# dflaxx/3d-hashjoin

Hardware: AMD Instinct MI355X
Metric: probe tuples/s + build ms, exp1 key/FK |R|=1e7 |S|=1e8, 1/2/4/8 GPU (higher is better)
Workload: dtype u32; 1 GPU; exp1 key/FK plan Csr, |R|=10000000 |S|=100000000 per GPU, uniform FKs, b=1; config=B, plan=Csr, R_total=10000000, S_total=100000000, R_per_gpu=10000000, S_per_gpu=100000000, num_buckets=10000000, emit_pairs=True, parallelism=single GPU, rehearsal_one_gpu=False

## Files before the change

3d-hashjoin_amd/csrc/radix.hip:

```cpp
#include <cmath>

#include "radix_seg.hpp"

namespace hj3d {
namespace {

constexpr int kPBlock = 1024;
constexpr int kPRounds = 16;
constexpr int kPTile = kPBlock * kPRounds;
constexpr int kPRoundsR = 8;
constexpr int kPSeg = 16;
__device__ __forceinline__ void put(uint2* p, uint2 e) { *p = e; }
__device__ __forceinline__ void put(uint32_t* p, uint32_t v) { *p = v; }
static_assert(kPTile == 1 << 14, "k_rp_scatter packs (partition, rank) as p << 14 | rank");
constexpr uint32_t kMaxParts = 2048;
constexpr uint32_t kBuildSlice = 16384;
constexpr uint32_t kSortedMax = 32;

struct FastDiv {
  uint64_t m;
  static FastDiv make(uint32_t d) {
    FastDiv f;
    f.m = ~uint64_t(0) / d + 1;
    f.d1 = d == 1;
    return f;
  }
  __device__ __forceinline__ uint32_t div(uint32_t a) const { return d1 ? a : uint32_t(__umul64hi(m, uint64_t(a))); }
  bool d1 = false;
};

struct RelTiles {
  RelView r0, r1;
  uint32_t nt0;
  uint32_t P;
  uint32_t tsz = kPTile;
  __device__ __forceinline__ bool second(uint32_t tile) const { return tile >= nt0; }
  __device__ __forceinline__ const RelView& rel(uint32_t tile) const { return tile >= nt0 ? r1 : r0; }
  __device__ __forceinline__ uint64_t base(uint32_t tile) const {
    return uint64_t(tile >= nt0 ? tile - nt0 : tile) * tsz;
  }
  __device__ __forceinline__ uint32_t pofs(uint32_t tile) const { return tile >= nt0 ? P : 0u; }
};

template <int ROUNDS>
__global__ __launch_bounds__(kPBlock) void k_rp_hist(RelTiles rt, FastMod fm, uint32_t lo, uint32_t nbl, FastDiv fw,
                                                     uint32_t P, uint32_t ntiles, uint32_t* __restrict__ hist,
                                                     uint32_t* __restrict__ cur) {
  __shared__ uint32_t cnt[kMaxParts];
  for (uint32_t p = threadIdx.x; p < P; p += kPBlock) cnt[p] = 0;
  __syncthreads();
  uint32_t key[ROUNDS];
  auto load = [&](uint32_t tile) __attribute__((always_inline)) {
    const RelView& r = rt.rel(tile);
    const uint64_t b = rt.base(tile);
#pragma unroll
    for (int j = 0; j < ROUNDS; ++j) {
      const uint64_t i = b + uint64_t(j) * kPBlock + threadIdx.x;
      key[j] = tile < ntiles && i < r.n ? r.key(i) : 0u;
    }
  };
  load(blockIdx.x);
  for (uint32_t tile = blockIdx.x; tile < ntiles; tile += gridDim.x) {
    const RelView& r = rt.rel(tile);
    const uint64_t b = rt.base(tile);
    const uint32_t pofs = rt.pofs(tile);
    uint32_t bl[ROUNDS];
#pragma unroll
    for (int j = 0; j < ROUNDS; ++j) {
      const uint64_t i = b + uint64_t(j) * kPBlock + threadIdx.x;
      bl[j] = i < r.n ? fm.mod(murmur32(key[j])) - lo : nbl;
    }
    load(tile + gridDim.x);
#pragma unroll
    for (int j = 0; j < ROUNDS; ++j)
      if (bl[j] < nbl) atomicAdd(&cnt[pofs + fw.div(bl[j])], 1u);
  }
  __syncthreads();
  for (uint32_t p = threadIdx.x; p < P; p += kPBlock) {
    const uint32_t c = cnt[p];
    hist[uint64_t(blockIdx.x) * P + p] = c ? atomicAdd(&cur[p], c) : 0u;
  }
}

template <int BLOCK = kJBlock>
__device__ uint32_t lds_excl_scan(uint32_t* a, uint32_t n, uint32_t* wsum);

template <int ROUNDS>
__global__ __launch_bounds__(kPBlock) void k_rp_scatter(RelTiles rt, FastMod fm, uint32_t lo, uint32_t nbl, FastDiv fw,
                                                        uint32_t P, uint32_t ntiles, const uint32_t* __restrict__ offs,
                                                        const uint32_t* __restrict__ cur, uint32_t* __restrict__ cur_next,
                                                        uint32_t* __restrict__ ps, uint2* __restrict__ out) {
  constexpr int kTile = kPBlock * ROUNDS;
  __shared__ uint2 stage[kTile];
  __shared__ uint32_t loc[kMaxParts];
  __shared__ uint32_t gb[kMaxParts];
  uint32_t* wsum = reinterpret_cast<uint32_t*>(stage);
  const bool explicit_rows = rt.r0.row_off != 0xFFFFFFFFu;
  uint32_t h[ROUNDS], rw[ROUNDS];
  auto load = [&](uint32_t tile) __attribute__((always_inline)) {
    const RelView& r = rt.rel(tile);
    const uint64_t b = rt.base(tile);
#pragma unroll
    for (int j = 0; j < ROUNDS; ++j) {
      const uint64_t i = b + uint64_t(j) * kPBlock + threadIdx.x;
      const bool ok = tile < ntiles && i < r.n;
      h[j] = ok ? r.key(i) : 0u;
      rw[j] = explicit_rows && ok ? r.row(i) : 0u;
    }
  };
  load(blockIdx.x);
  for (uint32_t p = threadIdx.x; p < P; p += kPBlock) gb[p] = cur[p];
  __syncthreads();
  const uint32_t total = lds_excl_scan<kPBlock>(gb, P, wsum);
  for (uint32_t p = threadIdx.x; p < P; p += kPBlock) {
    if (blockIdx.x == 0) ps[p] = gb[p];
    gb[p] += offs[uint64_t(blockIdx.x) * P + p];
  }
  if (blockIdx.x == 0) {
    if (threadIdx.x == 0) ps[P] = total;
    for (uint32_t p = threadIdx.x; p <= kMaxParts; p += kPBlock) cur_next[p] = 0;
  }
  for (uint32_t tile = blockIdx.x; tile < ntiles; tile += gridDim.x) {
    for (uint32_t p = threadIdx.x; p < P; p += kPBlock) loc[p] = 0;
    const RelView& r = rt.rel(tile);
    const uint64_t base = rt.base(tile);
    const uint32_t pofs = rt.pofs(tile);
    uint32_t rk[ROUNDS];
    __syncthreads();
#pragma unroll
    for (int j = 0; j < ROUNDS; ++j) {
      const uint64_t i = base + uint64_t(j) * kPBlock + threadIdx.x;
      h[j] = murmur32(h[j]);
      const uint32_t bl = fm.mod(h[j]) - lo;
      if (i < r.n && bl < nbl) {
        const uint32_t part = pofs + fw.div(bl);
        rk[j] = (part << 14) | atomicAdd(&loc[part], 1u);
      } else {
        rk[j] = kInvalid;
      }
    }
    __syncthreads();
    const uint32_t m = lds_excl_scan(loc, P, wsum);
#pragma unroll
    for (int j = 0; j < ROUNDS; ++j) {
      if (rk[j] == kInvalid) continue;
      const uint64_t i = base + uint64_t(j) * kPBlock + threadIdx.x;
      stage[loc[rk[j] >> 14] + (rk[j] & (kTile - 1))] = make_uint2(h[j], explicit_rows ? rw[j] : r.row(i));
    }
    __syncthreads();
    load(tile + gridDim.x);
    for (uint32_t k = threadIdx.x; k < m; k += kPBlock) {
      const uint2 e = stage[k];
      const uint32_t p = pofs + fw.div(fm.mod(e.x) - lo);
      put(out + gb[p] + (k - loc[p]), e);
    }
    __syncthreads();
    for (uint32_t p = threadIdx.x; p < P; p += kPBlock)
      gb[p] += (p + 1 < P ? loc[p + 1] : m) - loc[p];
    __syncthreads();
  }
}

constexpr int kFzRounds = 8;
constexpr int kFzGroup = 2;
constexpr int kFzTMax = 6;
struct FzBar {
  uint64_t* bar;
  uint64_t target;
  uint64_t* tflag;
  uint64_t tag;
  uint64_t ticks;
  uint32_t skip0;
};
__device__ __forceinline__ void grid_barrier(const FzBar& b) {
  __syncthreads();
  if (threadIdx.x == 0) {
    if (!(b.skip0 && blockIdx.x == 0)) __hip_atomic_fetch_add(b.bar, 1ull, __ATOMIC_RELEASE, __HIP_MEMORY_SCOPE_AGENT);
    const uint64_t t0 = wall_clock64();
    while (__hip_atomic_load(b.bar, __ATOMIC_ACQUIRE, __HIP_MEMORY_SCOPE_AGENT) < b.target) {
      __builtin_amdgcn_s_sleep(2);
      if (wall_clock64() - t0 > b.ticks) {
        __hip_atomic_store(b.bar + 1, 1ull, __ATOMIC_RELAXED, __HIP_MEMORY_SCOPE_AGENT);
        __hip_atomic_store(b.tflag, b.tag, __ATOMIC_RELAXED, __HIP_MEMORY_SCOPE_AGENT);
        break;
      }
    }
  }
  __syncthreads();
}

struct FzGeom {
  FastDiv32 dnb, dw;
  uint32_t nb, lo, nbl, P;
  __device__ __forceinline__ uint32_t bucket(uint32_t h) const { return h - dnb.div(h) * nb - lo; }
};
template <int TMAX>
__global__ __launch_bounds__(kPBlock) void k_rp_fused(RelTiles rt, FzGeom fz, uint32_t ntiles, uint32_t* __restrict__ cur,
                                                      uint32_t* __restrict__ cur_next, uint32_t* __restrict__ ps,
                                                      uint2* __restrict__ out, FzBar fb) {
  constexpr int R = kFzRounds;
  constexpr int kTile = kPBlock * R;
  __shared__ uint2 stage[kTile * kFzGroup];
  __shared__ uint32_t loc[kMaxParts];
  __shared__ uint32_t gb[kMaxParts];
  uint32_t* wsum = reinterpret_cast<uint32_t*>(stage);
  const uint32_t G = gridDim.x, P = fz.P, me = threadIdx.x;
  uint32_t hv[TMAX][R];
  for (uint32_t p = me; p < P; p += kPBlock) loc[p] = 0;
  const auto nleft = [&](uint32_t tile) __attribute__((always_inline)) {
    const RelView& r = rt.rel(tile);
    const uint64_t b = rt.base(tile);
    return tile < ntiles && r.n > b ? uint32_t(min(r.n - b, uint64_t(kTile))) : 0u;
  };
#pragma unroll
  for (int t = 0; t < TMAX; ++t) {
    const uint32_t tile = blockIdx.x + uint32_t(t) * G;
    const RelView& r = rt.rel(tile);
    const uint32_t nl = nleft(tile);
    const char* tb = r.base + rt.base(tile) * r.stride + r.key_off;
#pragma unroll
    for (int j = 0; j < R; ++j) {
      const uint32_t li = uint32_t(j) * kPBlock + me;
      hv[t][j] = li < nl ? (*reinterpret_cast<const uint32_t*>(tb + li * r.stride))
                         : 0u;
    }
  }
  __syncthreads();
#pragma unroll
  for (int t = 0; t < TMAX; ++t) {
    const uint32_t tile = blockIdx.x + uint32_t(t) * G;
    const uint32_t nl = nleft(tile), pofs = rt.pofs(tile);
#pragma unroll
    for (int j = 0; j < R; ++j) {
      hv[t][j] = murmur32(hv[t][j]);
      const uint32_t bl = fz.bucket(hv[t][j]);
      if (uint32_t(j) * kPBlock + me < nl && bl < fz.nbl) atomicAdd(&loc[pofs + fz.dw.div(bl)], 1u);
    }
  }
  __syncthreads();
  for (uint32_t p = me; p < P; p += kPBlock) {
    const uint32_t c = loc[p];
    gb[p] = c ? atomicAdd(&cur[p], c) : 0u;
  }
  grid_barrier(fb);
  for (uint32_t p = me; p < P; p += kPBlock) loc[p] = __hip_atomic_load(cur + p, __ATOMIC_RELAXED, __HIP_MEMORY_SCOPE_AGENT);
  __syncthreads();
  const uint32_t total = lds_excl_scan<kPBlock>(loc, P, wsum);
  for (uint32_t p = me; p < P; p += kPBlock) {
    if (blockIdx.x == 0) ps[p] = loc[p];
    gb[p] += loc[p];
  }
  if (blockIdx.x == 0) {
    if (me == 0) ps[P] = total;
    for (uint32_t p = me; p <= kMaxParts; p += kPBlock) cur_next[p] = 0;
  }
#pragma unroll
  for (int t0 = 0; t0 < TMAX; t0 += kFzGroup) {
    if (blockIdx.x + uint32_t(t0) * G >= ntiles) break;
    __syncthreads();
    for (uint32_t p = me; p < P; p += kPBlock) loc[p] = 0;
    uint32_t rk[kFzGroup][R];
    __syncthreads();
#pragma unroll
    for (int u = 0; u < kFzGroup; ++u) {
      const int t = t0 + u < TMAX ? t0 + u : TMAX - 1;
      const uint32_t nl = t0 + u < TMAX ? nleft(blockIdx.x + uint32_t(t) * G) : 0u;
#pragma unroll
      for (int j = 0; j < R; ++j) {
        asm volatile("" : "+v"(hv[t][j]));
        const uint32_t bl = fz.bucket(hv[t][j]);
        rk[u][j] = kInvalid;
        if (uint32_t(j) * kPBlock + me < nl && bl < fz.nbl) {
          const uint32_t part = fz.dw.div(bl);
          rk[u][j] = (part << 15) | atomicAdd(&loc[part], 1u);
        }
      }
    }
    __syncthreads();
    const uint32_t m = lds_excl_scan<kPBlock>(loc, P, wsum);
#pragma unroll
    for (int u = 0; u < kFzGroup; ++u) {
      const int t = t0 + u < TMAX ? t0 + u : TMAX - 1;
      const uint32_t rb = uint32_t(rt.r0.row_base + rt.base(blockIdx.x + uint32_t(t) * G));
#pragma unroll
      for (int j = 0; j < R; ++j) {
        if (rk[u][j] == kInvalid) continue;
        stage[loc[rk[u][j] >> 15] + (rk[u][j] & 0x7FFFu)] = make_uint2(hv[t][j], rb + uint32_t(j) * kPBlock + me);
      }
    }
    __syncthreads();
    for (uint32_t k = me; k < m; k += kPBlock) {
      const uint2 e = stage[k];
      const uint32_t p = fz.dw.div(fz.bucket(e.x));
      put(out + gb[p] + (k - loc[p]), e);
    }
    __syncthreads();
    for (uint32_t p = me; p < P; p += kPBlock) gb[p] += (p + 1 < P ? loc[p + 1] : m) - loc[p];
  }
}

constexpr uint32_t kRpWsMin = 4;
constexpr int kRpSmallRounds = 8;
constexpr int kWsRounds = 8;
constexpr int kWsSub = kPBlock * kWsRounds;
template <int PPT>
struct WsGeom {
  static constexpr uint32_t kSeg = PPT == 1 ? 16u : 8u;
  static constexpr uint32_t kStage = PPT == 1 ? 17408u : 15360u;
};
template <int PPT, bool EXPL>
__global__ __launch_bounds__(kPBlock) void k_rp_wscatter(RelTiles rt, FastMod fm, uint32_t lo, uint32_t nbl, FastDiv fw,
                                                         uint32_t P, uint32_t ntiles, const uint32_t* __restrict__ offs,
                                                         const uint32_t* __restrict__ cur, uint32_t* __restrict__ cur_next,
                                                         uint32_t* __restrict__ ps, uint2* __restrict__ out) {
  constexpr uint32_t SEG = WsGeom<PPT>::kSeg, STAGE = WsGeom<PPT>::kStage;
  __shared__ uint2 stage[STAGE];
  __shared__ uint32_t loc[kPBlock * PPT];
  __shared__ uint32_t sbase[kPBlock * PPT];
  __shared__ uint2 seginfo[STAGE / SEG];
  __shared__ uint32_t wsum[kPBlock / kWave];
  const uint32_t me = threadIdx.x;
  const int lane = threadIdx.x & 63, wid = threadIdx.x >> 6;
  for (uint32_t p = me; p < P; p += kPBlock) loc[p] = cur[p];
  __syncthreads();
  const uint32_t total = lds_excl_scan<kPBlock>(loc, P, wsum);
  if (blockIdx.x == 0) {
    for (uint32_t p = me; p < P; p += kPBlock) ps[p] = loc[p];
    if (me == 0) ps[P] = total;
    for (uint32_t p = me; p <= kMaxParts; p += kPBlock) cur_next[p] = 0;
  }
  uint32_t my_cur[PPT], my_kc[PPT], my_skip[PPT];
  uint2 creg[PPT][SEG - 1];
#pragma unroll
  for (int k = 0; k < PPT; ++k) {
    const uint32_t p = me + k * kPBlock;
    const uint32_t st = p < P ? loc[p] + offs[uint64_t(blockIdx.x) * P + p] : 0u;
    my_skip[k] = st % SEG;
    my_cur[k] = st - my_skip[k];
    my_kc[k] = my_skip[k];
#pragma unroll
    for (int j = 0; j < int(SEG) - 1; ++j) creg[k][j] = make_uint2(0, 0);
  }
  __syncthreads();
  for (uint32_t p = me; p < kPBlock * PPT; p += kPBlock) loc[p] = 0;
  __syncthreads();
  uint32_t h[kWsRounds], rw[EXPL ? kWsRounds : 1];
  auto load = [&](uint32_t tile, uint32_t hf) __attribute__((always_inline)) {
    const RelView& r = rt.rel(tile);
    const uint64_t base = rt.base(tile) + uint64_t(hf) * kWsSub;
#pragma unroll
    for (int j = 0; j < kWsRounds; ++j) {
      const uint64_t i = base + uint64_t(j) * kPBlock + me;
      h[j] = i < r.n ? r.key(i) : 0u;
      if constexpr (EXPL) rw[j] = i < r.n ? r.row(i) : 0u;
    }
  };
  auto flush_carry = [&]() __attribute__((always_inline)) {
#pragma unroll
    for (int k = 0; k < PPT; ++k) {
#pragma unroll
      for (int j = 0; j < int(SEG) - 1; ++j)
        if (uint32_t(j) < my_kc[k] && uint32_t(j) >= my_skip[k]) out[my_cur[k] + j] = creg[k][j];
      my_cur[k] += my_kc[k];
      my_kc[k] = 0;
      my_skip[k] = 0;
    }
  };
  auto scan = [&](uint32_t v, uint32_t* tot) __attribute__((always_inline)) {
    uint32_t wt;
    const uint32_t pre = wave_excl_scan(v, &wt);
    if (lane == 0) wsum[wid] = wt;
    __syncthreads();
    uint32_t base = 0, all = 0;
#pragma unroll
    for (int w = 0; w < kPBlock / kWave; ++w) {
      const uint32_t t = wsum[w];
      base += w < wid ? t : 0u;
      all += t;
    }
    __syncthreads();
    *tot = all;
    return base + pre;
  };
  auto process = [&](uint32_t tile, uint32_t hf, uint32_t ntile, uint32_t nhf) __attribute__((always_inline)) {
    const RelView& r = rt.rel(tile);
    const uint64_t base = rt.base(tile) + uint64_t(hf) * kWsSub;
    const uint32_t pofs = rt.pofs(tile);
    uint32_t rk[kWsRounds];
#pragma unroll
    for (int j = 0; j < kWsRounds; ++j) {
      const uint64_t i = base + uint64_t(j) * kPBlock + me;
      h[j] = murmur32(h[j]);
      const uint32_t bl = fm.mod(h[j]) - lo;
      rk[j] = kInvalid;
      if (i < r.n && bl < nbl) {
        const uint32_t p = pofs + fw.div(bl);
        rk[j] = (p << 13) | atomicAdd(&loc[p], 1u);
      }
    }
    __syncthreads();
    uint32_t c[PPT], L[PPT], pack = 0;
#pragma unroll
    for (int k = 0; k < PPT; ++k) {
      const uint32_t p = me + k * kPBlock;
      c[k] = p < P ? loc[p] : 0u;
      loc[p] = 0;
      L[k] = my_kc[k] + c[k];
      pack += (L[k] << 16) | (L[k] / SEG);
    }
    uint32_t tot;
    uint32_t pre = scan(pack, &tot);
    if ((tot >> 16) > STAGE) {
      flush_carry();
      pack = 0;
#pragma unroll
      for (int k = 0; k < PPT; ++k) {
        L[k] = c[k];
        pack += (L[k] << 16) | (L[k] / SEG);
      }
      pre = scan(pack, &tot);
    }
    const uint32_t nfull = tot & 0xFFFFu;
    uint32_t at = pre >> 16, fseg = pre & 0xFFFFu;
#pragma unroll
    for (int k = 0; k < PPT; ++k) {
      const uint32_t p = me + k * kPBlock;
      if (p < P) {
        sbase[p] = at + my_kc[k];
#pragma unroll
        for (int j = 0; j < int(SEG) - 1; ++j)
          if (uint32_t(j) < my_kc[k]) stage[at + j] = creg[k][j];
        for (uint32_t sg = 0; sg < L[k] / SEG; ++sg)
          seginfo[fseg + sg] = make_uint2(my_cur[k] + sg * SEG, (at + sg * SEG) | ((sg == 0 ? my_skip[k] : 0u) << 16));
      }
      at += L[k];
      fseg += L[k] / SEG;
    }
    __syncthreads();
#pragma unroll
    for (int j = 0; j < kWsRounds; ++j) {
      if (rk[j] == kInvalid) continue;
      const uint64_t i = base + uint64_t(j) * kPBlock + me;
      uint32_t row;
      if constexpr (EXPL) row = rw[j];
      else row = uint32_t(r.row_base + i);
      stage[sbase[rk[j] >> 13] + (rk[j] & (kWsSub - 1))] = make_uint2(h[j], row);
    }
    if (ntile < ntiles) load(ntile, nhf);
    __syncthreads();
    for (uint32_t kk = me; kk < nfull * SEG; kk += kPBlock) {
      const uint2 si = seginfo[kk / SEG];
      const uint32_t j = kk % SEG;
      const uint2 e = stage[(si.y & 0xFFFFu) + j];
      if (j >= (si.y >> 16)) put(out + si.x + j, e);
    }
    at = pre >> 16;
#pragma unroll
    for (int k = 0; k < PPT; ++k) {
      const uint32_t F = L[k] - L[k] % SEG;
#pragma unroll
      for (int j = 0; j < int(SEG) - 1; ++j)
        if (uint32_t(j) < L[k] - F) creg[k][j] = stage[at + F + j];
      if (F) my_skip[k] = 0;
      my_cur[k] += F;
      my_kc[k] = L[k] - F;
      at += L[k];
    }
  };
  if (blockIdx.x < ntiles) load(blockIdx.x, 0);
  for (uint32_t tile = blockIdx.x; tile < ntiles; tile += gridDim.x) {
    process(tile, 0, tile, 1);
    process(tile, 1, tile + gridDim.x, 0);
  }
  flush_carry();
}

template <int BLOCK>
__device__ uint32_t lds_excl_scan(uint32_t* a, uint32_t n, uint32_t* wsum) {
  const uint32_t per = (n + BLOCK - 1) / BLOCK;
  const uint32_t beg = threadIdx.x * per;
  const uint32_t end = min(beg + per, n);
  uint32_t local = 0;
  for (uint32_t k = beg; k < end; ++k) local += a[k];
  const int lane = threadIdx.x & 63, wid = threadIdx.x >> 6;
  uint32_t x = local;
#pragma unroll
  for (int o = 1; o < 64; o <<= 1) {
    const uint32_t y = __shfl_up(x, o, kWave);
    if (lane >= o) x += y;
  }
  if (lane == 63) wsum[wid] = x;
  __syncthreads();
  uint32_t wpre = 0, tot = 0;
  for (int w = 0; w < BLOCK / kWave; ++w) {
    const uint32_t v = wsum[w];
    if (w < wid) wpre += v;
    tot += v;
  }
  uint32_t run = wpre + x - local;
  for (uint32_t k = beg; k < end; ++k) {
    const uint32_t v = a[k];
    a[k] = run;
    run += v;
  }
  __syncthreads();
  return tot;
}

__global__ __launch_bounds__(kJBlock) void k_rp_build(const uint2* __restrict__ pairs, const uint32_t* __restrict__ ps,
                                                      FastMod fm, uint32_t lo, uint32_t nbl, uint32_t W,
                                                      uint32_t* __restrict__ off, uint2* __restrict__ ent) {
  __shared__ uint32_t cnt[kBuildSlice];
  __shared__ uint32_t wsum[kJBlock / kWave];
  const uint32_t p = blockIdx.x;
  const uint32_t b0 = p * W;
  const uint32_t nbs = min(W, nbl - b0);
  const uint32_t s0 = ps[p], s1 = ps[p + 1];
  for (uint32_t k = threadIdx.x; k < nbs; k += kJBlock) cnt[k] = 0;
  __syncthreads();
  for (uint32_t i = s0 + threadIdx.x; i < s1; i += kJBlock) atomicAdd(&cnt[fm.mod(pairs[i].x) - lo - b0], 1u);
  __syncthreads();
  lds_excl_scan(cnt, nbs, wsum);
  for (uint32_t k = threadIdx.x; k < nbs; k += kJBlock) off[b0 + k] = s0 + cnt[k];
  if (b0 + nbs == nbl && threadIdx.x == 0) off[nbl] = s1;
  __syncthreads();
  for (uint32_t i = s0 + threadIdx.x; i < s1; i += kJBlock) {
    const uint2 e = pairs[i];
    const uint32_t pos = atomicAdd(&cnt[fm.mod(e.x) - lo - b0], 1u);
    ent[s0 + pos] = e;
  }
}

constexpr uint32_t kBuildSlice2 = 8192;
constexpr uint32_t kBuildSlice2Max = 10240;
constexpr uint32_t kBuildStage = 14400;

constexpr int kB3Per = 12;
template <int BLOCK, uint32_t WMAX, uint32_t STAGE>
__global__ __launch_bounds__(BLOCK) void k_rp_build3(const uint2* __restrict__ pairs, const uint32_t* __restrict__ ps,
                                                     FastMod fm, uint32_t lo, uint32_t nbl, uint32_t W, uint32_t P,
                                                     uint32_t* __restrict__ off, uint2* __restrict__ ent) {
  __shared__ uint32_t cnt[WMAX + 1];
  __shared__ uint2 stage[STAGE];
  __shared__ uint32_t wsum[BLOCK / kWave];
  constexpr uint32_t kCap = kB3Per * BLOCK;
  static_assert(kCap <= STAGE, "a register-held partition must fit the stage");
  uint2 ea[kB3Per], eb[kB3Per];
  auto load = [&](uint2 (&e)[kB3Per], uint32_t p) __attribute__((always_inline)) {
    if (p >= P) return;
    const uint32_t s0 = ps[p], s1 = ps[p + 1];
    if (s1 - s0 > kCap) return;
#pragma unroll
    for (int u = 0; u < kB3Per; ++u) {
      const uint32_t i = s0 + u * BLOCK + threadIdx.x;
      e[u] = i < s1 ? pairs[i] : make_uint2(0, 0);
    }
  };
  auto build = [&](uint2 (&e)[kB3Per], uint32_t p) __attribute__((always_inline)) {
    const uint32_t b0 = p * W;
    const uint32_t nbs = min(W, nbl - b0);
    const uint32_t s0 = ps[p], s1 = ps[p + 1], m = s1 - s0;
    for (uint32_t k = threadIdx.x; k < nbs; k += BLOCK) cnt[k] = 0;
    __syncthreads();
    if (m > kCap) {
      for (uint32_t i = s0 + threadIdx.x; i < s1; i += BLOCK) atomicAdd(&cnt[fm.mod(pairs[i].x) - lo - b0], 1u);
      __syncthreads();
      lds_excl_scan<BLOCK>(cnt, nbs, wsum);
      for (uint32_t k = threadIdx.x; k < nbs; k += BLOCK) off[b0 + k] = s0 + cnt[k];
      if (b0 + nbs == nbl && threadIdx.x == 0) off[nbl] = s1;
      __syncthreads();
      for (uint32_t i = s0 + threadIdx.x; i < s1; i += BLOCK) {
        const uint2 x = pairs[i];
        ent[s0 + atomicAdd(&cnt[fm.mod(x.x) - lo - b0], 1u)] = x;
      }
      __syncthreads();
      for (uint32_t k = threadIdx.x; k < nbs; k += BLOCK) {
        const uint32_t bs = k ? cnt[k - 1] : 0u, n = cnt[k] - bs;
        if (n < 2 || n > kSortedMax) continue;
        uint2* E = ent + s0 + bs;
        for (uint32_t q = 1; q < n; ++q) {
          const uint2 x = E[q];
          uint32_t j = q;
          while (j > 0 && E[j - 1].y > x.y) {
            E[j] = E[j - 1];
            --j;
          }
          E[j] = x;
        }
      }
      __syncthreads();
      return;
    }
    uint32_t rk[kB3Per];
#pragma unroll
    for (int u = 0; u < kB3Per; ++u) {
      const bool v = u * BLOCK + threadIdx.x < m;
      const uint32_t b = v ? fm.mod(e[u].x) - lo - b0 : 0u;
      rk[u] = v ? (b << 16) | atomicAdd(&cnt[b], 1u) : kInvalid;
    }
    __syncthreads();
    lds_excl_scan<BLOCK>(cnt, nbs, wsum);
    if (threadIdx.x == 0) cnt[nbs] = m;
    for (uint32_t k = threadIdx.x; k < nbs; k += BLOCK) put(off + b0 + k, s0 + cnt[k]);
    if (b0 + nbs == nbl && threadIdx.x == 0) off[nbl] = s1;
    __syncthreads();
#pragma unroll
    for (int u = 0; u < kB3Per; ++u)
      if (rk[u] != kInvalid) stage[cnt[rk[u] >> 16] + (rk[u] & 0xFFFFu)] = e[u];
    __syncthreads();
    for (uint32_t q = threadIdx.x; q < m; q += BLOCK) {
      const uint2 x = stage[q];
      const uint32_t b = fm.mod(x.x) - lo - b0;
      const uint32_t bs = cnt[b], n = cnt[b + 1] - bs;
      uint32_t pos = q;
      if (n >= 2 && n <= kSortedMax) {
        uint32_t r = 0;
        for (uint32_t k = bs; k < bs + n; ++k) r += stage[k].y < x.y;
        pos = bs + r;
      }
      put(ent + s0 + pos, x);
    }
    __syncthreads();
  };
  load(ea, blockIdx.x);
  for (uint32_t p = blockIdx.x; p < P; p += 2 * gridDim.x) {
    load(eb, p + gridDim.x);
    build(ea, p);
    if (p + gridDim.x >= P) break;
    load(ea, p + 2 * gridDim.x);
    build(eb, p + gridDim.x);
  }
}

enum Mode { kAgg = 0, kDense = 1, kCount = 2, kWrite = 3 };

template <bool UNIQUE, int MODE, bool CK, typename EntT>
__device__ __forceinline__ void probe_bucket(uint32_t h, uint32_t pr, const EntT* E, uint32_t s, uint32_t n,
                                             uint64_t (&acc)[kProbeFields], uint64_t i, uint2* __restrict__ out,
                                             uint64_t out_cap, uint64_t* __restrict__ cnt) {
  if (MODE != kWrite) acc[0] += 1;
  if (UNIQUE) {
    uint32_t match = kInvalid, cmps = 0;
    if (n <= kSortedMax) {
      cmps = n;
      for (uint32_t c = 0; c < n; ++c) {
        const uint2 e = E[s + (c == 0 ? 0u : n - c)];
        if (e.x == h) {
          cmps = c + 1;
          match = e.y;
          break;
        }
      }
    } else {
      uint32_t minrow = kInvalid, lo_m = kInvalid, hi_m = 0, nm = 0;
      for (uint32_t k = s; k < s + n; ++k) {
        const uint2 e = E[k];
        minrow = min(minrow, e.y);
        if (e.x == h) {
          ++nm;
          lo_m = min(lo_m, e.y);
          hi_m = max(hi_m, e.y);
        }
      }
      if (nm == 0) {
        cmps = n;
      } else if (lo_m == minrow) {
        cmps = 1;
        match = lo_m;
      } else {
        uint32_t gt = 0;
        for (uint32_t k = s; k < s + n; ++k) gt += E[k].y > hi_m;
        cmps = 2 + gt;
        match = hi_m;
      }
    }
    if (MODE != kWrite) acc[3] += cmps;
    if (MODE == kDense) {
      if (i < out_cap)
        __builtin_nontemporal_store((uint64_t(match) << 32) | pr, reinterpret_cast<uint64_t*>(out + i));
    }
    if (match != kInvalid) {
      if (MODE == kWrite) {
        const uint64_t o = cnt[i];
        if (o < out_cap) out[o] = make_uint2(pr, match);
      } else {
        acc[1] += 1;
        acc[2] += 1;
        if (CK) {
          acc[4] += pr;
          acc[5] += match;
          const uint64_t ph = pair_hash(pr, match);
          acc[7] += ph;
          acc[8] ^= ph;
        }
      }
    }
    if (MODE == kCount) cnt[i] = match != kInvalid;
  } else {
    if (MODE != kWrite) acc[3] += n;
    uint64_t o = (MODE == kWrite) ? cnt[i] : 0;
    uint32_t nout = 0;
    for (uint32_t k = s; k < s + n; ++k) {
      const uint2 e = E[k];
      if (e.x != h) continue;
      ++nout;
      if (MODE == kWrite) {
        if (o < out_cap) out[o] = make_uint2(pr, e.y);
        ++o;
      } else if (CK) {
        acc[4] += pr;
        acc[5] += e.y;
        const uint64_t ph = pair_hash(pr, e.y);
        acc[7] += ph;
        acc[8] ^= ph;
      }
    }
    if (MODE != kWrite) {
      acc[1] += nout != 0;
      acc[2] += nout;
    }
    if (MODE == kCount) cnt[i] = nout;
  }
}

template <int MODE, bool CK, int NG>
__device__ __forceinline__ void probe_group_unique(const uint64_t (&v)[kSegItems], const uint64_t (&slot)[kSegItems],
                                                   uint32_t valid, int g, const uint32_t* loff, const uint2* lent,
                                                   FastMod fm, uint32_t lob0, uint64_t (&acc)[kProbeFields],
                                                   uint2* __restrict__ out, uint64_t out_cap) {
  static_assert(MODE == kDense || MODE == kAgg, "unique dense / aggregate forms only");
  uint32_t d[NG], match[NG], cmps[NG];
  bool live[NG];
#pragma unroll
  for (int j = 0; j < NG; ++j) {
    const bool ok = (valid >> (g + j)) & 1u;
    const uint32_t w = loff[ok ? fm.mod(uint32_t(v[g + j])) - lob0 : 0u];
    d[j] = ok ? w : 0u;
  }
#pragma unroll
  for (int j = 0; j < NG; ++j) {
    const uint32_t n = d[j] & 0xFFFFu;
    match[j] = kInvalid;
    cmps[j] = n;
    live[j] = n != 0 && n <= kSortedMax;
  }
#pragma unroll
  for (uint32_t c = 0; c < 3; ++c) {
    uint2 e[NG];
#pragma unroll
    for (int j = 0; j < NG; ++j) {
      const uint32_t n = d[j] & 0xFFFFu;
      const bool ok = live[j] && c < n;
      e[j] = lent[ok ? (d[j] >> 16) + (c == 0 ? 0u : n - c) : 0u];
      const bool hit = ok && e[j].x == uint32_t(v[g + j]);
      match[j] = hit ? e[j].y : match[j];
      cmps[j] = hit ? c + 1 : cmps[j];
      live[j] = live[j] && !hit;
    }
  }
#pragma unroll
  for (int j = 0; j < NG; ++j) {
    const uint32_t h = uint32_t(v[g + j]), n = d[j] & 0xFFFFu, s = d[j] >> 16;
    if (live[j] && n > 3) {
      for (uint32_t c = 3; c < n; ++c) {
        const uint2 e = lent[s + n - c];
        if (e.x == h) {
          cmps[j] = c + 1;
          match[j] = e.y;
          break;
        }
      }
    } else if (n > kSortedMax) {
      uint32_t minrow = kInvalid, lo_m = kInvalid, hi_m = 0, nm = 0;
      for (uint32_t k = s; k < s + n; ++k) {
        const uint2 e = lent[k];
        minrow = min(minrow, e.y);
        if (e.x == h) {
          ++nm;
          lo_m = min(lo_m, e.y);
          hi_m = max(hi_m, e.y);
        }
      }
      if (nm != 0 && lo_m == minrow) {
        cmps[j] = 1;
        match[j] = lo_m;
      } else if (nm != 0) {
        uint32_t gt = 0;
        for (uint32_t k = s; k < s + n; ++k) gt += lent[k].y > hi_m;
        cmps[j] = 2 + gt;
        match[j] = hi_m;
      }
    }
  }
  uint32_t nv = 0, nm = 0, sc = 0;
#pragma unroll
  for (int j = 0; j < NG; ++j) {
    const bool ok = (valid >> (g + j)) & 1u;
    const uint32_t pr = uint32_t(v[g + j] >> 32);
    nv += ok;
    sc += cmps[j];
    const bool m = match[j] != kInvalid;
    nm += m;
    if (MODE == kDense && ok && slot[g + j] < out_cap)
      __builtin_nontemporal_store((uint64_t(match[j]) << 32) | pr, reinterpret_cast<uint64_t*>(out + slot[g + j]));
    if (CK && m) {
      acc[4] += pr;
      acc[5] += match[j];
      const uint64_t ph = pair_hash(pr, match[j]);
      acc[7] += ph;
      acc[8] ^= ph;
    }
  }
  acc[0] += nv;
  acc[1] += nm;
  acc[2] += nm;
  acc[3] += sc;
}

template <int MODE, bool CK, int NG = 4>
__device__ __forceinline__ void probe_chunk_unique(const uint64_t (&v)[kSegItems], const uint64_t (&slot)[kSegItems],
                                                   uint32_t valid, const uint32_t* loff, const uint2* lent,
                                                   FastMod fm, uint32_t lob0, uint64_t (&acc)[kProbeFields],
                                                   uint2* __restrict__ out, uint64_t out_cap) {
  static_assert(kSegItems % NG == 0, "groups of NG items");
#pragma unroll
  for (int g = 0; g < kSegItems; g += NG)
    probe_group_unique<MODE, CK, NG>(v, slot, valid, g, loff, lent, fm, lob0, acc, out, out_cap);
}
__device__ __forceinline__ void stage_slice(const uint32_t* __restrict__ off, const uint2* __restrict__ ent, uint32_t b0,
                                            uint32_t nbs, uint32_t e0, uint32_t ne, uint32_t* ldir, uint2* lent) {
  constexpr int kStage = 12;
  const uint64_t* src = reinterpret_cast<const uint64_t*>(ent + e0);
  uint64_t* dst = reinterpret_cast<uint64_t*>(lent);
  const uint32_t nmax = max(nbs, ne);
  for (uint32_t k0 = threadIdx.x; k0 < nmax; k0 += kJBlock * kStage) {
    uint32_t v[kStage], w[kStage];
    uint64_t x[kStage];
#pragma unroll
    for (int u = 0; u < kStage; ++u) {
      const uint32_t k = k0 + u * kJBlock;
      v[u] = k < nbs ? off[b0 + k] : 0u;
      w[u] = k < nbs ? off[b0 + k + 1] : 0u;
      x[u] = k < ne ? src[k] : 0ull;
    }
#pragma unroll
    for (int u = 0; u < kStage; ++u) {
      const uint32_t k = k0 + u * kJBlock;
      if (k < nbs) ldir[k] = ((v[u] - e0) << 16) | (w[u] - v[u]);
      if (k < ne) dst[k] = x[u];
    }
  }
}

template <int BLOCK, int ROUNDS, int MAXP, bool IMPLICIT>
__global__ __launch_bounds__(BLOCK) void k_rp_part1(RelView r, FastMod fm, uint32_t lo, uint32_t nbl, FastDiv fw,
                                                    uint32_t P, uint32_t ntiles, uint32_t cap,
                                                    uint2* __restrict__ region, uint32_t* __restrict__ counts,
                                                    uint2* __restrict__ ovf, unsigned long long* __restrict__ novf) {
  constexpr int TILE = BLOCK * ROUNDS;
  constexpr int TBITS = __builtin_ctz(TILE);
  static_assert((TILE & (TILE - 1)) == 0 && TILE <= (1 << 16), "tile must be a power of two");
  static_assert(MAXP < (1 << 16), "partition ids are packed into 16 bits");
  __shared__ uint2 stage[TILE];
  __shared__ uint32_t loc[MAXP + 1];
  __shared__ uint32_t cur[MAXP];
  __shared__ uint32_t wsum[BLOCK / kWave];
  const uint64_t gbase = uint64_t(blockIdx.x) * P;
  for (uint32_t p = threadIdx.x; p < P; p += BLOCK) cur[p] = 0;
  uint32_t h[ROUNDS];
  uint32_t rw[IMPLICIT ? 1 : ROUNDS];
#pragma unroll
  for (int j = 0; j < ROUNDS; ++j) {
    const uint64_t i = uint64_t(blockIdx.x) * TILE + uint64_t(j) * BLOCK + threadIdx.x;
    h[j] = i < r.n ? r.key(i) : 0u;
    if constexpr (!IMPLICIT) rw[j] = i < r.n ? r.row(i) : 0u;
  }
  const int lane = threadIdx.x & 63;
  const uint64_t lt = lane == 0 ? 0ull : (~0ull >> (64 - lane));
  for (uint32_t tile = blockIdx.x; tile < ntiles; tile += gridDim.x) {
    for (uint32_t p = threadIdx.x; p < P; p += BLOCK) loc[p] = 0;
    const uint64_t base = uint64_t(tile) * TILE;
    uint32_t rk[ROUNDS];
    __syncthreads();
#pragma unroll
    for (int j = 0; j < ROUNDS; ++j) {
      const uint64_t i = base + uint64_t(j) * BLOCK + threadIdx.x;
      h[j] = murmur32(h[j]);
      const uint32_t bl = fm.mod(h[j]) - lo;
      if (i < r.n && bl < nbl) {
        const uint32_t part = fw.div(bl);
        rk[j] = (part << TBITS) | atomicAdd(&loc[part], 1u);
      } else {
        rk[j] = kInvalid;
      }
    }
    __syncthreads();
    const uint32_t m = lds_excl_scan<BLOCK>(loc, P, wsum);
    if (threadIdx.x == 0) loc[P] = m;
#pragma unroll
    for (int j = 0; j < ROUNDS; ++j) {
      if (rk[j] == kInvalid) continue;
      const uint32_t li = uint32_t(j) * BLOCK + threadIdx.x;
      uint32_t y = ((rk[j] >> TBITS) << 16) | li;
      if constexpr (!IMPLICIT) y = rw[j];
      stage[loc[rk[j] >> TBITS] + (rk[j] & (TILE - 1))] = make_uint2(h[j], y);
    }
    __syncthreads();
    const uint64_t nbase = uint64_t(tile + gridDim.x) * TILE;
#pragma unroll
    for (int j = 0; j < ROUNDS; ++j) {
      const uint64_t i = nbase + uint64_t(j) * BLOCK + threadIdx.x;
      h[j] = i < r.n ? r.key(i) : 0u;
      if constexpr (!IMPLICIT) rw[j] = i < r.n ? r.row(i) : 0u;
    }
    constexpr int kOutU = 4;
    for (uint32_t k0 = 0; k0 < m; k0 += kOutU * BLOCK) {
      uint2 e[kOutU];
      uint32_t o[kOutU], p[kOutU];
#pragma unroll
      for (int u = 0; u < kOutU; ++u) {
        const uint32_t k = k0 + u * BLOCK + threadIdx.x;
        e[u] = k < m ? stage[k] : make_uint2(0, 0);
      }
#pragma unroll
      for (int u = 0; u < kOutU; ++u) {
        const uint32_t k = k0 + u * BLOCK + threadIdx.x;
        if (IMPLICIT) {
          p[u] = e[u].y >> 16;
          e[u].y = uint32_t(r.row_base + base) + (e[u].y & 0xFFFFu);
        } else {
          p[u] = fw.div(fm.mod(e[u].x) - lo);
        }
        o[u] = k < m ? cur[p[u]] + (k - loc[p[u]]) : 0u;
      }
// ... 670 lines not shown
```

Baseline: 121.2 billion probe tuples/s.

## Rank all tiles once in fused partition kernel and overlap local scan with grid barrier

The fused radix-partition kernel now records each element's block-local rank during the first counting pass, packed as 16-bit slots in registers. It splits the grid barrier into arrive and wait so the local exclusive scan and slot finalisation run while other workgroups arrive. The old per-group recount and rescan is replaced by scattering into the shared stage through fixed-size windows. It also adds compile-time-disabled wall-clock instrumentation in the fused and build kernels. The cost is more register pressure from the packed slot arrays and an extra LDS array for global starts.

```diff
diff --git a/3d-hashjoin_amd/csrc/radix.hip b/3d-hashjoin_amd/csrc/radix.hip
--- a/3d-hashjoin_amd/csrc/radix.hip
+++ b/3d-hashjoin_amd/csrc/radix.hip
@@ -16,6 +16,35 @@
 constexpr uint32_t kMaxParts = 2048;
 constexpr uint32_t kBuildSlice = 16384;
 constexpr uint32_t kSortedMax = 32;
+
+#ifndef HJ3D_RP_CLK
+#define HJ3D_RP_CLK 0
+#endif
+constexpr int kRpClkPts = 32;
+#if HJ3D_RP_CLK
+#define RP_CLK_DECL __shared__ uint64_t rp_clk[kRpClkPts]
+#define RP_CLK(i)                                   \
+  do {                                              \
+    if (threadIdx.x == 0) rp_clk[i] = wall_clock64(); \
+  } while (0)
+#define RP_CLK_SYNC(i)                                 \
+  do {                                                 \
+    asm volatile("s_waitcnt vmcnt(0) lgkmcnt(0)" ::: "memory"); \
+    __syncthreads();                                   \
+    RP_CLK(i);                                         \
+  } while (0)
+#define RP_CLK_PRINT(name, npts)                                                                      \
+  do {                                                                                                \
+    if (threadIdx.x == 0 && (blockIdx.x == 0 || blockIdx.x == gridDim.x / 2))                         \
+      for (int q = 0; q < (npts); ++q)                                                                \
+        printf("rpclk %s wg %u pt %d %llu\n", name, blockIdx.x, q, (unsigned long long)rp_clk[q]);     \
+  } while (0)
+#else
+#define RP_CLK_DECL
+#define RP_CLK(i)
+#define RP_CLK_SYNC(i)
+#define RP_CLK_PRINT(name, npts)
+#endif
 
 struct FastDiv {
   uint64_t m;
@@ -162,8 +191,9 @@
 }
 
 constexpr int kFzRounds = 8;
-constexpr int kFzGroup = 2;
+constexpr uint32_t kFzWin = 16384;
 constexpr int kFzTMax = 6;
+constexpr uint32_t kFzNone = 0xFFFFu;
 struct FzBar {
   uint64_t* bar;
   uint64_t target;
@@ -172,10 +202,13 @@
   uint64_t ticks;
   uint32_t skip0;
 };
-__device__ __forceinline__ void grid_barrier(const FzBar& b) {
+__device__ __forceinline__ void grid_arrive(const FzBar& b) {
   __syncthreads();
+  if (threadIdx.x == 0 && !(b.skip0 && blockIdx.x == 0))
+    __hip_atomic_fetch_add(b.bar, 1ull, __ATOMIC_RELEASE, __HIP_MEMORY_SCOPE_AGENT);
+}
+__device__ __forceinline__ void grid_wait(const FzBar& b) {
   if (threadIdx.x == 0) {
-    if (!(b.skip0 && blockIdx.x == 0)) __hip_atomic_fetch_add(b.bar, 1ull, __ATOMIC_RELEASE, __HIP_MEMORY_SCOPE_AGENT);
     const uint64_t t0 = wall_clock64();
     while (__hip_atomic_load(b.bar, __ATOMIC_ACQUIRE, __HIP_MEMORY_SCOPE_AGENT) < b.target) {
       __builtin_amdgcn_s_sleep(2);
@@ -200,12 +233,19 @@
                                                       uint2* __restrict__ out, FzBar fb) {
   constexpr int R = kFzRounds;
   constexpr int kTile = kPBlock * R;
-  __shared__ uint2 stage[kTile * kFzGroup];
+  static_assert(R % 2 == 0 && uint32_t(TMAX) * kTile <= 3 * kFzWin && 3 * kFzWin <= kFzNone,
+                "slots fit 16 bits and three windows; kFzNone >> 14 names no window");
+  __shared__ uint2 stage[kFzWin];
   __shared__ uint32_t loc[kMaxParts];
   __shared__ uint32_t gb[kMaxParts];
+  __shared__ uint32_t gs[kMaxParts];
+  __shared__ uint32_t dump[kWave];
   uint32_t* wsum = reinterpret_cast<uint32_t*>(stage);
   const uint32_t G = gridDim.x, P = fz.P, me = threadIdx.x;
   uint32_t hv[TMAX][R];
+  uint32_t sl[TMAX][R / 2];
+  RP_CLK_DECL;
+  RP_CLK(0);
   for (uint32_t p = me; p < P; p += kPBlock) loc[p] = 0;
   const auto nleft = [&](uint32_t tile) __attribute__((always_inline)) {
     const RelView& r = rt.rel(tile);
@@ -226,77 +266,96 @@
     }
   }
   __syncthreads();
+  RP_CLK_SYNC(1);
 #pragma unroll
   for (int t = 0; t < TMAX; ++t) {
-    const uint32_t tile = blockIdx.x + uint32_t(t) * G;
-    const uint32_t nl = nleft(tile), pofs = rt.pofs(tile);
+    const uint32_t nl = nleft(blockIdx.x + uint32_t(t) * G);
+    uint32_t rk[R];
 #pragma unroll
     for (int j = 0; j < R; ++j) {
       hv[t][j] = murmur32(hv[t][j]);
       const uint32_t bl = fz.bucket(hv[t][j]);
-      if (uint32_t(j) * kPBlock + me < nl && bl < fz.nbl) atomicAdd(&loc[pofs + fz.dw.div(bl)], 1u);
-    }
+      const bool ok = uint32_t(j) * kPBlock + me < nl && bl < fz.nbl;
+      rk[j] = atomicAdd(ok ? &loc[fz.dw.div(bl)] : &dump[me % kWave], 1u);
+      rk[j] = ok ? rk[j] : kFzNone;
+    }
+#pragma unroll
+    for (int j = 0; j < R; j += 2) {
+      sl[t][j / 2] = rk[j] | rk[j + 1] << 16;
+      asm volatile("" : "+v"(sl[t][j / 2]));
+    }
+    __builtin_amdgcn_sched_barrier(0);
   }
   __syncthreads();
+  RP_CLK(2);
   for (uint32_t p = me; p < P; p += kPBlock) {
     const uint32_t c = loc[p];
     gb[p] = c ? atomicAdd(&cur[p], c) : 0u;
   }
-  grid_barrier(fb);
-  for (uint32_t p = me; p < P; p += kPBlock) loc[p] = __hip_atomic_load(cur + p, __ATOMIC_RELAXED, __HIP_MEMORY_SCOPE_AGENT);
+  RP_CLK_SYNC(3);
+  grid_arrive(fb);
+  const uint32_t m = lds_excl_scan<kPBlock>(loc, P, wsum);
+#pragma unroll
+  for (int t = 0; t < TMAX; ++t) {
+    uint32_t ls[R];
+#pragma unroll
+    for (int j = 0; j < R; ++j) {
+      asm volatile("" : "+v"(hv[t][j]));
+      const uint32_t s = j & 1 ? sl[t][j / 2] >> 16 : sl[t][j / 2] & 0xFFFFu;
+      ls[j] = loc[s != kFzNone ? fz.dw.div(fz.bucket(hv[t][j])) : 0u];
+    }
+#pragma unroll
+    for (int j = 0; j < R; j += 2) {
+      const uint32_t w = sl[t][j / 2], s0 = w & 0xFFFFu, s1 = w >> 16;
+      sl[t][j / 2] = (s0 != kFzNone ? s0 + ls[j] : s0) | (s1 != kFzNone ? s1 + ls[j + 1] : s1) << 16;
+      asm volatile("" : "+v"(sl[t][j / 2]));
+    }
+    __builtin_amdgcn_sched_barrier(0);
+  }
+  RP_CLK(4);
+  grid_wait(fb);
+  RP_CLK(5);
+  for (uint32_t p = me; p < P; p += kPBlock) gs[p] = __hip_atomic_load(cur + p, __ATOMIC_RELAXED, __HIP_MEMORY_SCOPE_AGENT);
   __syncthreads();
-  const uint32_t total = lds_excl_scan<kPBlock>(loc, P, wsum);
+  const uint32_t total = lds_excl_scan<kPBlock>(gs, P, wsum);
   for (uint32_t p = me; p < P; p += kPBlock) {
-    if (blockIdx.x == 0) ps[p] = loc[p];
-    gb[p] += loc[p];
+    const uint32_t s = gs[p];
+    if (blockIdx.x == 0) ps[p] = s;
+    gb[p] += s - loc[p];
   }
   if (blockIdx.x == 0) {
     if (me == 0) ps[P] = total;
     for (uint32_t p = me; p <= kMaxParts; p += kPBlock) cur_next[p] = 0;
   }
-#pragma unroll
-  for (int t0 = 0; t0 < TMAX; t0 += kFzGroup) {
-    if (blockIdx.x + uint32_t(t0) * G >= ntiles) break;
-    __syncthreads();
-    for (uint32_t p = me; p < P; p += kPBlock) loc[p] = 0;
-    uint32_t rk[kFzGroup][R];
-    __syncthreads();
-#pragma unroll
-    for (int u = 0; u < kFzGroup; ++u) {
-      const int t = t0 + u < TMAX ? t0 + u : TMAX - 1;
-      const uint32_t nl = t0 + u < TMAX ? nleft(blockIdx.x + uint32_t(t) * G) : 0u;
+  RP_CLK(6);
+  for (uint32_t w = 0; w * kFzWin < m; ++w) {
+    if (w) __syncthreads();
+    uint32_t mew = me;
+    asm volatile("" : "+v"(mew));
+#pragma unroll
+    for (int t = 0; t < TMAX; ++t) {
+      const uint32_t rb = uint32_t(rt.r0.row_base + rt.base(blockIdx.x + uint32_t(t) * G));
 #pragma unroll
       for (int j = 0; j < R; ++j) {
-        asm volatile("" : "+v"(hv[t][j]));
-        const uint32_t bl = fz.bucket(hv[t][j]);
-        rk[u][j] = kInvalid;
-        if (uint32_t(j) * kPBlock + me < nl && bl < fz.nbl) {
-          const uint32_t part = fz.dw.div(bl);
-          rk[u][j] = (part << 15) | atomicAdd(&loc[part], 1u);
-        }
-      }
-    }
-    __syncthreads();
-    const uint32_t m = lds_excl_scan<kPBlock>(loc, P, wsum);
-#pragma unroll
-    for (int u = 0; u < kFzGroup; ++u) {
-      const int t = t0 + u < TMAX ? t0 + u : TMAX - 1;
-      const uint32_t rb = uint32_t(rt.r0.row_base + rt.base(blockIdx.x + uint32_t(t) * G));
-#pragma unroll
-      for (int j = 0; j < R; ++j) {
-        if (rk[u][j] == kInvalid) continue;
-        stage[loc[rk[u][j] >> 15] + (rk[u][j] & 0x7FFFu)] = make_uint2(hv[t][j], rb + uint32_t(j) * kPBlock + me);
-      }
-    }
-    __syncthreads();
-    for (uint32_t k = me; k < m; k += kPBlock) {
+        if (!(j & 1)) asm volatile("" : "+v"(sl[t][j / 2]));
+        const uint32_t s = j & 1 ? sl[t][j / 2] >> 16 : sl[t][j / 2] & 0xFFFFu;
+        uint32_t h = hv[t][j];
+        asm volatile("" : "+v"(h));
+        if (s / kFzWin == w) stage[s % kFzWin] = make_uint2(h, rb + uint32_t(j) * kPBlock + mew);
+      }
+      __builtin_amdgcn_sched_barrier(0);
+    }
+    __syncthreads();
+    RP_CLK(7 + 2 * w);
+    const uint32_t wb = w * kFzWin, mw = min(m - wb, kFzWin);
+    for (uint32_t k = me; k < mw; k += kPBlock) {
       const uint2 e = stage[k];
-      const uint32_t p = fz.dw.div(fz.bucket(e.x));
-      put(out + gb[p] + (k - loc[p]), e);
-    }
-    __syncthreads();
-    for (uint32_t p = me; p < P; p += kPBlock) gb[p] += (p + 1 < P ? loc[p + 1] : m) - loc[p];
-  }
+      put(out + gb[fz.dw.div(fz.bucket(e.x))] + wb + k, e);
+    }
+    RP_CLK(8 + 2 * w);
+  }
+  RP_CLK_SYNC(15);
+  RP_CLK_PRINT("fused", 16);
 }
 
 constexpr uint32_t kRpWsMin = 4;
@@ -546,6 +605,9 @@
   constexpr uint32_t kCap = kB3Per * BLOCK;
   static_assert(kCap <= STAGE, "a register-held partition must fit the stage");
   uint2 ea[kB3Per], eb[kB3Per];
+  RP_CLK_DECL;
+  [[maybe_unused]] int ck = 0;
+  RP_CLK(ck++);
   auto load = [&](uint2 (&e)[kB3Per], uint32_t p) __attribute__((always_inline)) {
     if (p >= P) return;
     const uint32_t s0 = ps[p], s1 = ps[p + 1];
@@ -562,6 +624,7 @@
     const uint32_t s0 = ps[p], s1 = ps[p + 1], m = s1 - s0;
     for (uint32_t k = threadIdx.x; k < nbs; k += BLOCK) cnt[k] = 0;
     __syncthreads();
+    RP_CLK(ck < 31 ? ck++ : 31);
     if (m > kCap) {
       for (uint32_t i = s0 + threadIdx.x; i < s1; i += BLOCK) atomicAdd(&cnt[fm.mod(pairs[i].x) - lo - b0], 1u);
       __syncthreads();
@@ -599,15 +662,19 @@
       rk[u] = v ? (b << 16) | atomicAdd(&cnt[b], 1u) : kInvalid;
     }
     __syncthreads();
+    RP_CLK(ck < 31 ? ck++ : 31);
     lds_excl_scan<BLOCK>(cnt, nbs, wsum);
+    RP_CLK(ck < 31 ? ck++ : 31);
     if (threadIdx.x == 0) cnt[nbs] = m;
     for (uint32_t k = threadIdx.x; k < nbs; k += BLOCK) put(off + b0 + k, s0 + cnt[k]);
     if (b0 + nbs == nbl && threadIdx.x == 0) off[nbl] = s1;
     __syncthreads();
+    RP_CLK(ck < 31 ? ck++ : 31);
 #pragma unroll
     for (int u = 0; u < kB3Per; ++u)
       if (rk[u] != kInvalid) stage[cnt[rk[u] >> 16] + (rk[u] & 0xFFFFu)] = e[u];
     __syncthreads();
+    RP_CLK(ck < 31 ? ck++ : 31);
     for (uint32_t q = threadIdx.x; q < m; q += BLOCK) {
       const uint2 x = stage[q];
       const uint32_t b = fm.mod(x.x) - lo - b0;
@@ -621,6 +688,7 @@
       put(ent + s0 + pos, x);
     }
     __syncthreads();
+    RP_CLK(ck < 31 ? ck++ : 31);
   };
   load(ea, blockIdx.x);
   for (uint32_t p = blockIdx.x; p < P; p += 2 * gridDim.x) {
@@ -630,6 +698,8 @@
     load(ea, p + 2 * gridDim.x);
     build(eb, p + gridDim.x);
   }
+  RP_CLK_SYNC(31);
+  RP_CLK_PRINT("build3", kRpClkPts);
 }
 
 enum Mode { kAgg = 0, kDense = 1, kCount = 2, kWrite = 3 };
```

Result: no change. 121.1 billion probe tuples/s (-0.1%).
